# Medical-Image-Analysis-Laboratory/fetal_t2mapping

Measured on AMD Instinct MI355X. Metric: Mvoxel/s T2 fit, 256³×8TE 3-param LM, 1/2/4/8 GPU; % HBM roofline, higher is better.
Workload: dtype f64

## Files before the change

### fetal_t2mapping_amd/csrc/t2fit_boot.hip

```cpp
#include <hip/hip_runtime.h>

#include <chrono>
#include <cmath>
#include <cstdint>
#include <cstdio>
#include <cstdlib>
#include <mutex>
#include <string>
#include <vector>

#include "t2fit_config.h"
#include "t2fit_context.h"
#include "t2fit_error.h"
#include "t2fit_support.h"

namespace {

using t2fit::kBlock;
constexpr int kMaxIntervalReplicas = 512;

__device__ inline void philox4x32_10(uint32_t c0, uint32_t c1, uint32_t c2, uint32_t c3, uint32_t k0, uint32_t k1,
                                     uint32_t& w0, uint32_t& w1) {
#pragma unroll
  for (int round = 0; round < 10; ++round) {
// ... 243 lines not shown
  long long c = 0;
  for (int64_t v = (int64_t)blockIdx.x * kBlock + threadIdx.x; v < n_vox; v += (int64_t)kBgBlocks * kBlock) {
    if (mask[v] != 0) continue;
    for (int j = 0; j < n_te; ++j) {
      const double x = (double)(layout == T2FIT_LAYOUT_TE_MAJOR ? echoes[(int64_t)j * n_vox + v] : echoes[v * n_te + j]);
      s += x * x;
    }
    c += n_te;
  }
  bg_block_reduce(s, c, sh_s, sh_c, part_sum, part_cnt, blockIdx.x);
}

__global__ __launch_bounds__(kBlock) void boot_background_final_kernel(const double* part_sum, const long long* part_cnt,
                                                                       double* out_sum, long long* out_cnt) {
  __shared__ double sh_s[kBlock];
  __shared__ long long sh_c[kBlock];
  double s = 0.0;
  long long c = 0;
  for (int i = threadIdx.x; i < kBgBlocks; i += kBlock) {
    s += part_sum[i];
    c += part_cnt[i];
  }
  bg_block_reduce(s, c, sh_s, sh_c, out_sum, out_cnt, 0);
}

using t2fit::aligned16;
using t2fit::fail;

#ifdef T2FIT_BOOT_PHASES
struct Phases {
  std::chrono::steady_clock::time_point t = std::chrono::steady_clock::now();
  void mark(const char* name) {
    const auto now = std::chrono::steady_clock::now();
    fprintf(stderr, "[t2fit boot phase] %-28s %9.3f ms\n", name, std::chrono::duration<double, std::milli>(now - t).count());
    t = now;
  }
};
#else
struct Phases {
  void mark(const char*) {}
};
#endif

struct BootWorkspace {
  std::vector<void*> dev;
  hipStream_t streams[2] = {nullptr, nullptr};
  bool own_streams = false;
  std::vector<hipEvent_t> events;
  ~BootWorkspace() {
    Phases ph;
    for (hipStream_t s : streams)
      if (s) (void)hipStreamSynchronize(s);
    for (hipEvent_t e : events) (void)hipEventDestroy(e);
    if (own_streams)
      for (hipStream_t s : streams)
        if (s) (void)hipStreamDestroy(s);
    ph.mark("release: sync, events, streams");
    for (void* p : dev) (void)hipFree(p);
    ph.mark("release: hipFree");
  }
  hipError_t alloc(void** p, size_t bytes) {
    const hipError_t e = hipMalloc(p, bytes ? bytes : 16);
    if (e == hipSuccess) dev.push_back(*p);
    return e;
  }
  hipError_t event(hipEvent_t* e) {
    const hipError_t rc = hipEventCreateWithFlags(e, hipEventDisableTiming);
    if (rc == hipSuccess) events.push_back(*e);
    return rc;
  }
};

std::string gib(double bytes) {
  char b[48];
  snprintf(b, sizeof b, "%.2f GiB", bytes / (1024.0 * 1024.0 * 1024.0));
  return b;
}

int synth_check(const char* who, const t2fit_config* cfg, const float* t2_dev, const float* k_dev, double noise_scalar,
                const float* noise_map_dev, int64_t n_vox, int noise_kind) {
  const char* why;
  const int rc = t2fit::config_check(cfg, &why);
  if (rc != T2FIT_OK) return fail(rc, std::string(who) + ": " + why);
  if (cfg->norm)
    return fail(T2FIT_E_INVALID, std::string(who) + ": cfg.norm = 1 is not supported (the maps of a normalised fit are in "
                                 "per-voxel units of the largest sample, and the noise level would have to be too)");
  if (!t2_dev || !k_dev) return fail(T2FIT_E_INVALID, std::string(who) + ": t2_dev / k_dev is NULL");
  if (n_vox < 1 || n_vox >= (1LL << 32)) return fail(T2FIT_E_INVALID, std::string(who) + ": n_vox must be in 1..2^32-1");
  if (noise_kind != T2FIT_BOOT_NOISE_RICIAN && noise_kind != T2FIT_BOOT_NOISE_GAUSSIAN)
    return fail(T2FIT_E_INVALID, std::string(who) + ": unknown noise_kind");
  if (!noise_map_dev && !(noise_scalar >= 0.0 && noise_scalar <= 3.0e38))
    return fail(T2FIT_E_INVALID, std::string(who) + ": noise_scalar must be finite and >= 0 (or give noise_map_dev)");
  return T2FIT_OK;
}

int synth_launch(const t2fit_config* cfg, const float* t2_dev, const float* k_dev, double noise_scalar,
                 const float* noise_map_dev, const uint8_t* mask_dev, int64_t n_vox, int64_t voxel_offset, uint64_t seed,
                 int replica, int noise_kind, float* out, hipStream_t st) {
  SynthArgs a{};
  a.t2 = t2_dev; a.k = k_dev; a.noise_map = noise_map_dev; a.mask = mask_dev; a.out = out;
  a.n_vox = n_vox;
  a.voxel_offset = (uint64_t)voxel_offset;
  a.key0 = (uint32_t)seed; a.key1 = (uint32_t)(seed >> 32); a.replica = (uint32_t)replica;
  a.n_te = cfg->n_te;
  a.noise_scalar = (float)noise_scalar;
  for (int j = 0; j < cfg->n_te; ++j) a.te[j] = (float)cfg->te_ms[j];
  const bool vec = n_vox % 4 == 0 && aligned16(t2_dev) && aligned16(k_dev) && aligned16(out) &&
                   (!noise_map_dev || aligned16(noise_map_dev)) && (reinterpret_cast<uintptr_t>(mask_dev) & 3u) == 0;
  const bool rician = noise_kind == T2FIT_BOOT_NOISE_RICIAN;
// ... 256 lines not shown
```

### fetal_t2mapping_amd/csrc/t2fit_dispatch.h

```cpp
#pragma once

#include "t2fit_lane.h"
#include "t2fit_lbfgsb.h"
#include "t2fit_lm.h"
#include "t2fit_loglin.h"

namespace t2fit {

inline LaneParams make_lane_params(const t2fit_config& c) {
  LaneParams P;
  P.model = c.model; P.solver = c.solver; P.precision = c.precision; P.n_te = c.n_te;
  P.no_prior = c.no_prior; P.norm = c.norm; P.maxls = c.maxls; P.maxiter = c.maxiter;
  P.maxfun = c.maxfun; P.numpy_legacy = c.numpy_legacy != 0;
  for (int i = 0; i < T2FIT_MAX_TE; ++i) {
    P.te[i] = i < c.n_te ? c.te_ms[i] : 0.0;
    P.te_f[i] = (float)P.te[i];
  }
  for (int j = 0; j < 3; ++j) { P.x0[j] = c.x0[j]; P.lb[j] = c.lb[j]; P.ub[j] = c.ub[j]; }
  P.ftol = c.ftol; P.gtol = c.gtol; P.fd_step = c.fd_step; P.lm_xtol = c.lm_xtol;
  P.np_k_ub = c.noprior_k_ub; P.np_t2_lb = c.noprior_t2_lb; P.np_t2_ub = c.noprior_t2_ub;
  P.lm_r_lo = 1.0 / (c.no_prior ? c.noprior_t2_ub : c.ub[1]);
  P.lm_r_hi = 1.0 / (c.no_prior ? c.noprior_t2_lb : c.lb[1]);
  P.lm_r_x0 = 1.0 / c.x0[1];
  t2_exp_res_coefficients(P.exp_c);
  P.inv_n = 1.0 / c.n_te;
  P.te_max = 0.0;
  for (int i = 0; i < c.n_te; ++i) P.te_max = c.te_ms[i] > P.te_max ? c.te_ms[i] : P.te_max;
  P.lbfgsb_tol = (c.ftol / 2.220446049250313e-16) * 2.220446049250313e-16;
  return P;
}

struct LaneOutputs {
  float t2, k, sigma, res, r2, fun, se;
  int32_t nit;
  uint8_t status;
};

T2_HD ObjCtx prepare_samples(const LaneParams& P, float* col, int stride, bool& finite, float& y0_raw) {
  const int n = P.n_te;
  finite = true;
  y0_raw = col[0];
  float ymax = col[0];
  for (int i = 0; i < n; ++i) {
    const float v = col[i * stride];
    finite = finite && t2_finite(v);
    ymax = v > ymax ? v : ymax;
  }
  if (P.norm) {
    for (int i = 0; i < n; ++i) {
      const float v = col[i * stride] / ymax;
      col[i * stride] = v;
      finite = finite && t2_finite(v);
    }
  }
  ObjCtx c;
  c.P = &P;
  c.y = EchoView{col, stride};
  return c;
}

template <int SOLVER, int PREC, int MODEL>
T2_HD void fit_lane_t(const LaneParams& P, const ObjCtx& c, bool finite, float y0_raw, LaneResult& r) {
  constexpr int NP = MODEL == T2FIT_MODEL_GAUSSIAN ? 2 : 3;
  double lb[3], ub[3];
  const bool feasible = lane_bounds(P, y0_raw, lb, ub);
  r.nit = 0;
  r.nfev = 0;
  r.fun = NAN;
  if (!feasible) {
    r.x[0] = r.x[1] = NAN;
    r.x[2] = NP == 2 ? 0.0 : NAN;
    r.status = T2FIT_ST_INFEASIBLE;
    return;
  }
  if (!finite) {
    for (int j = 0; j < 3; ++j) r.x[j] = j < NP ? t2_clip(P.x0[j], lb[j], ub[j]) : 0.0;
    r.status = T2FIT_ST_NONFINITE;
    return;
  }
  if constexpr (SOLVER == T2FIT_SOLVER_LOGLIN) {
    static_assert(MODEL == T2FIT_MODEL_GAUSSIAN, "the log-linear closed form exists for the 2-parameter model only");
    loglin_solve(c, lb, ub, true, r);
  } else if constexpr (SOLVER == T2FIT_SOLVER_LM) {
    static_assert(MODEL != T2FIT_MODEL_RICIAN, "LM handles the least-squares models only");
    if constexpr (PREC == T2FIT_PREC_F32) lm_solve<float, NP>(c, lb, ub, r);
    else lm_solve<double, NP>(c, lb, ub, r);
  } else {
    lbfgsb_solve<MODEL>(c, lb, ub, r);
  }
}

T2_HD float r_squared(const ObjCtx& c, double k, double t2, double sg) {
  const LaneParams& P = *c.P;
  const int n = P.n_te;
  double mean = 0.0;
  for (int i = 0; i < n; ++i) mean += (double)c.sample(i);
  mean /= n;
  double ss_tot = 0.0, ss_res = 0.0;
  const bool sq = P.model == T2FIT_MODEL_GAUSSIAN_RICIAN;
  for (int i = 0; i < n; ++i) {
    const double yi = (double)c.sample(i);
    const double E = t2_exp(-P.te[i] / t2);
    const double m = sq ? t2_sqrt(k * k * E * E + sg * sg) : k * E;
    ss_res += (yi - m) * (yi - m);
    ss_tot += (yi - mean) * (yi - mean);
  }
  return (float)(1.0 - ss_res / ss_tot);
}

T2_HD float t2_std_error(const ObjCtx& c, double k, double t2, double sg) {
  const LaneParams& P = *c.P;
  const int n = P.n_te;
  const bool sq = P.model == T2FIT_MODEL_GAUSSIAN_RICIAN;
  const int np = P.model == T2FIT_MODEL_GAUSSIAN ? 2 : 3;
  if (n <= np) return NAN;
  double a00 = 0, a01 = 0, a02 = 0, a11 = 0, a12 = 0, a22 = 0, ss = 0;
  for (int i = 0; i < n; ++i) {
    const double t = P.te[i];
    const double E = t2_exp(-t / t2);
    double m, jk, jt, js;
    if (sq) {
      m = t2_sqrt(k * k * E * E + sg * sg);
      jk = k * E * E / m;
      jt = k * k * E * E * (t / (t2 * t2)) / m;
      js = sg / m;
    } else {
      m = k * E;
      jk = E;
      jt = m * t / (t2 * t2);
      js = 0.0;
    }
    const double r = (double)c.sample(i) - m;
    ss += r * r;
    a00 += jk * jk; a01 += jk * jt; a02 += jk * js; a11 += jt * jt; a12 += jt * js; a22 += js * js;
  }
  const double s2 = ss / (n - np);
  double var;
  if (sq) {
    const double det = a00 * (a11 * a22 - a12 * a12) - a01 * (a01 * a22 - a12 * a02) + a02 * (a01 * a12 - a11 * a02);
    var = s2 * (a00 * a22 - a02 * a02) / det;
  } else if (np == 3) {
    var = s2 * a00 / (a00 * a11 - a01 * a01);
  } else {
    var = s2 * a00 / (a00 * a11 - a01 * a01);
  }
  return var > 0.0 ? (float)t2_sqrt(var) : NAN;
}

T2_HD void lane_epilogue(const ObjCtx& c, const LaneResult& r, LaneOutputs& o, bool want_r2, bool want_se) {
  o.k = (float)r.x[0];
  o.t2 = (float)r.x[1];
  o.sigma = (float)r.x[2];
  o.fun = (float)r.fun;
  o.nit = r.nit;
  o.status = r.status;
  o.res = residual_mean(c, o.k, o.t2, o.sigma);
  o.r2 = want_r2 ? r_squared(c, (double)o.k, (double)o.t2, (double)o.sigma) : 0.0f;
  o.se = want_se ? t2_std_error(c, (double)o.k, (double)o.t2, (double)o.sigma) : 0.0f;
}

}
```

### fetal_t2mapping_amd/csrc/t2fit_kernels.hip

```cpp
#include <hip/hip_runtime.h>

#include <algorithm>
#include <atomic>
#include <cstdlib>
#include <string>

#include "t2fit_config.h"
#include "t2fit_diag.h"
#include "t2fit_dispatch.h"
#include "t2fit_error.h"
#include "t2fit_launch.h"
#include "t2fit_support.h"

using namespace t2fit;

namespace {

constexpr int kLdsStride = kBlock + 1;
#ifndef T2_SAMPLE_LOAD
#define T2_SAMPLE_LOAD(p) (*(p))
#endif
#ifndef T2_WAVE_HINT
#define T2_WAVE_HINT 2
#endif
constexpr int kWaveHint = T2_WAVE_HINT;

struct Tuning {
  bool use_persistent = true;
  int persistent_blocks = 2048;
  int refill_min = 0;
  bool nte_special = true;
  int take = 0;
  int64_t small_volume = 1 << 20;
  int wave_wg = 1;
  int waves_per_cu = 0;
};
std::atomic<bool> g_reserve_set{false};
std::atomic<int> g_reserve_cus{0};

const Tuning& tuning() {
  static const Tuning tuned = [] {
    Tuning t;
    if (const char* e = std::getenv("T2FIT_ONE_SHOT")) t.use_persistent = std::atoi(e) == 0;
    if (const char* e = std::getenv("T2FIT_PERSISTENT_BLOCKS")) t.persistent_blocks = std::max(1, std::atoi(e));
    if (const char* e = std::getenv("T2FIT_REFILL_MIN")) t.refill_min = std::min(64, std::max(1, std::atoi(e)));
    if (const char* e = std::getenv("T2FIT_RESERVE_CUS"); e && !g_reserve_set.load()) g_reserve_cus.store(std::max(0, std::atoi(e)));
    if (const char* e = std::getenv("T2FIT_NTE_SPECIAL")) t.nte_special = std::atoi(e) != 0;
    if (const char* e = std::getenv("T2FIT_TAKE")) t.take = std::max(0, std::min(64, std::atoi(e)));
    if (const char* e = std::getenv("T2FIT_SMALL_VOLUME")) t.small_volume = std::max<int64_t>(0, std::atoll(e));
    if (const char* e = std::getenv("T2FIT_WAVE_WG")) t.wave_wg = std::max(0, std::atoi(e));
    if (const char* e = std::getenv("T2FIT_WAVES_PER_CU")) t.waves_per_cu = std::max(0, std::atoi(e));
    return t;
  }();
  return tuned;
}

thread_local bool g_timing = false;
constexpr int kEvRing = 16;
thread_local hipEvent_t g_ev0[kEvRing] = {}, g_ev1[kEvRing] = {}, g_ev2[kEvRing] = {};
thread_local long g_ev_count = 0;
thread_local int g_ev_slot = 0;

double event_ms(int launches_ago, const hipEvent_t* from, const hipEvent_t* to) {
  if (launches_ago < 0 || launches_ago >= kEvRing || launches_ago >= g_ev_count) return -1.0;
  const int slot = (int)((g_ev_count - 1 - launches_ago) % kEvRing);
  if (hipEventSynchronize(to[slot]) != hipSuccess) return -1.0;
  float ms = 0.0f;
  if (hipEventElapsedTime(&ms, from[slot], to[slot]) != hipSuccess) return -1.0;
  return (double)ms;
}

struct DevMaps {
  float *t2, *k, *sigma, *res, *r2, *fun, *se;
  int32_t* nit;
  uint8_t* status;
  double* xd;
  double* fund;
  double* trace = nullptr;
  int32_t* trace_len = nullptr;
  int trace_cap = 0;
};

__device__ __forceinline__ void stage_echoes(float* lds, const float* __restrict__ echoes, int layout,
                                             int n_te, int64_t n_vox, int64_t base, bool load_own) {
  const int lane = threadIdx.x;
  if (layout == T2FIT_LAYOUT_TE_MAJOR) {
    if (load_own) {
      const float* src = echoes + base + lane;
      for (int i = 0; i < n_te; ++i) lds[i * kLdsStride + lane] = src[(int64_t)i * n_vox];
    }
  } else {
    const int64_t rows = n_vox - base < kBlock ? n_vox - base : kBlock;
    const int total = (int)rows * n_te;
    const float* src = echoes + base * n_te;
    for (int j = lane; j < total; j += kBlock) {
      const int v = j / n_te;
      const int i = j - v * n_te;
      lds[i * kLdsStride + v] = src[j];
    }
    __syncthreads();
  }
}

template <bool kExtras = true, bool kEpilogueFollows = false>
__device__ __forceinline__ void store_masked(const DevMaps& m, int64_t v) {
  m.t2[v] = 0.0f; m.k[v] = 0.0f; m.sigma[v] = 0.0f;
  if constexpr (!kEpilogueFollows) m.res[v] = 0.0f;
  if constexpr (!kExtras) return;
// ... 457 lines not shown
        busy = false;
        done = true;
      }
    }
  }
  if (done) {
    LaneResult r;
    A::result(s, c, r);
    store_fit<kExtras>(m, v, r);
  }
  T2_STAMPS_END(next_chunk, lane)
}

template <class A, int kChunk, bool kTrace = false, int kWavesPerSimd = 1, bool kExtras = true, int kWg = kBlock,
          bool kRegs = false>
__global__ __launch_bounds__(kWg, kWavesPerSimd) void fit_persistent_kernel(const LaneParams P,
                                                                    const float* __restrict__ echoes, int layout,
                                                                    const uint8_t* __restrict__ mask, int64_t n_vox,
                                                                    DevMaps m, unsigned long long* next_chunk, int refill_min,
                                                                    int take, double* ghist) {
  persistent_fit<A, kChunk, kTrace, kExtras, kWg, kRegs>(P, echoes, layout, mask, n_vox, m, next_chunk, refill_min, take, ghist,
                                                         (KernargParams)__builtin_amdgcn_kernarg_segment_ptr());
}

__global__ __launch_bounds__(kBlock) void residuals_kernel(const LaneParams P, const float* __restrict__ echoes,
                                                           int layout, const uint8_t* __restrict__ mask,
                                                           int64_t n_vox, const float* __restrict__ t2,
                                                           const float* __restrict__ k,
                                                           const float* __restrict__ sigma, float* res, float* r2,
                                                           float* se) {
  extern __shared__ float lds[];
  const int lane = threadIdx.x;
  const int64_t base = (int64_t)blockIdx.x * kBlock;
  const int64_t v = base + lane;
  const bool in_range = v < n_vox;
  const bool active = in_range && (mask == nullptr || mask[v] != 0);
  stage_echoes(lds, echoes, layout, P.n_te, n_vox, base, active);
  if (!in_range) return;
  float out = 0.0f, out2 = 0.0f, out3 = 0.0f;
  if (active) {
    bool finite;
    float y0_raw;
    const ObjCtx c = prepare_samples(P, lds + lane, kLdsStride, finite, y0_raw);
    const float kv = k[v], tv = t2[v], sv = sigma ? sigma[v] : 0.0f;
    out = residual_mean(c, kv, tv, sv);
    if (r2) out2 = r_squared(c, (double)kv, (double)tv, (double)sv);
    if (se) out3 = t2_std_error(c, (double)kv, (double)tv, (double)sv);
  }
  res[v] = out;
  if (r2) r2[v] = out2;
  if (se) se[v] = out3;
}

using FitKernel = void (*)(const LaneParams, const float*, int, const uint8_t*, int64_t, DevMaps);

FitKernel pick_kernel(const t2fit_config& c) {
  if (c.solver == T2FIT_SOLVER_LM) {
    if (c.precision == T2FIT_PREC_F32)
      return c.model == T2FIT_MODEL_GAUSSIAN
                 ? fit_volume_kernel<T2FIT_SOLVER_LM, T2FIT_PREC_F32, T2FIT_MODEL_GAUSSIAN>
                 : fit_volume_kernel<T2FIT_SOLVER_LM, T2FIT_PREC_F32, T2FIT_MODEL_GAUSSIAN_RICIAN>;
    return c.model == T2FIT_MODEL_GAUSSIAN
               ? fit_volume_kernel<T2FIT_SOLVER_LM, T2FIT_PREC_F64, T2FIT_MODEL_GAUSSIAN>
               : fit_volume_kernel<T2FIT_SOLVER_LM, T2FIT_PREC_F64, T2FIT_MODEL_GAUSSIAN_RICIAN>;
  }
  if (c.solver == T2FIT_SOLVER_LOGLIN)
    return fit_volume_kernel<T2FIT_SOLVER_LOGLIN, T2FIT_PREC_F64, T2FIT_MODEL_GAUSSIAN>;
  return nullptr;
}

bool wants_extras(const DevMaps& dm) { return dm.r2 || dm.se || dm.fun || dm.nit || dm.status || dm.xd || dm.fund; }

struct LaunchArgs {
  unsigned grid; size_t lds_samples; hipStream_t st;
  const LaneParams& P; const float* echoes; int layout; const uint8_t* mask; int64_t n_vox; const DevMaps& dm;
  unsigned long long* counter;
  bool big;
};

template <class A, bool kLargeOnly = false, bool kWaveOnly = false>
hipError_t launch_persistent(const LaunchArgs& a) {
  constexpr int W = A::kWavesPerSimd;
  const Tuning& tune = tuning();
  const DevMaps& dm = a.dm;
  const bool extras = wants_extras(dm);
  const int refill_min = tune.refill_min > 0 ? tune.refill_min : A::kRefillMin;
  if constexpr (!kPhaseStamps && kLargeOnly && A::kHistDoubles > 0 && A::kWaveWgOk) {
    if (tune.wave_wg) {
      using AW = typename A::WaveWg;
      constexpr int kHint = AW::kWaveWgHint;
      auto k64 = extras ? fit_persistent_kernel<AW, kChunkSmall, false, kHint, true, 64, true>
                        : fit_persistent_kernel<AW, kChunkSmall, false, kHint, false, 64, true>;
      unsigned wg = 64;
      if constexpr (kWgShapeDiag) {
        if (tune.wave_wg == 2) { k64 = fit_persistent_kernel<AW, kChunkSmall, false, 1, false, 256, true>; wg = 256; }
        if (tune.wave_wg == 3) { k64 = fit_persistent_kernel<AW, kChunkSmall, false, 1, false, 128, true>; wg = 128; }
      }
      size_t lds64 = (size_t)AW::kHistDoubles * wg * sizeof(double);
      unsigned per_cu = (unsigned)std::min<size_t>(wg == 64 ? 4 * kHint : 512 / wg, 128 / ceil_div<size_t>(lds64, 1280));
      if (tune.waves_per_cu > 0 && (unsigned)tune.waves_per_cu < per_cu) {
        per_cu = (unsigned)tune.waves_per_cu;
        lds64 = (size_t)(128 / per_cu) * 1280;
      }
      hipError_t e = hipFuncSetAttribute(reinterpret_cast<const void*>(k64), hipFuncAttributeMaxDynamicSharedMemorySize,
                                         (int)lds64);
      if (e != hipSuccess) return e;
// ... 15 lines not shown
    return hipErrorNotSupported;
  } else {
    auto kern = extras ? fit_persistent_kernel<A, kChunkLarge, false, W, true>
                       : fit_persistent_kernel<A, kChunkLarge, false, W, false>;
    if constexpr (!kLargeOnly) {
      if (dm.trace) kern = fit_persistent_kernel<A, kChunkSmall, true, W>;
      else if (!a.big) kern = fit_persistent_kernel<A, kChunkSmall, false, W>;
    }
    const size_t lds = ((a.lds_samples / sizeof(float) + 1) & ~(size_t)1) * sizeof(float) +
                       (size_t)A::kHistDoubles * kBlock * sizeof(double) +
                       (size_t)(kBlock / 64) * (kQueueCap * sizeof(uint32_t) + kStampLdsBytesPerWave);
    hipError_t e = hipFuncSetAttribute(reinterpret_cast<const void*>(kern), hipFuncAttributeMaxDynamicSharedMemorySize,
                                       (int)lds);
    if (e != hipSuccess) return e;
    hipLaunchKernelGGL(kern, dim3(a.grid), dim3(kBlock), lds, a.st, a.P, a.echoes, a.layout, a.mask, a.n_vox, dm, a.counter,
                       refill_min, 1, (double*)nullptr);
    return hipGetLastError();
  }
}

template <int MODEL>
hipError_t launch_lbfgsb(int n_te, const LaunchArgs& a) {
  if (a.big && tuning().nte_special) {
    if (n_te == 8) return launch_persistent<LbfgsbLane<MODEL, 8>, true>(a);
    if (n_te == 6) return launch_persistent<LbfgsbLane<MODEL, 6>, true>(a);
    if (n_te == 3) return launch_persistent<LbfgsbLane<MODEL, 3>, true>(a);
    hipError_t e = hipErrorNotSupported;
    if (tuning().wave_wg == 1) {
      if (n_te == 7) e = launch_persistent<LbfgsbLane<MODEL, 7>, true, true>(a);
      if (n_te == 5) e = launch_persistent<LbfgsbLane<MODEL, 5>, true, true>(a);
      if (n_te == 4) e = launch_persistent<LbfgsbLane<MODEL, 4>, true, true>(a);
    }
    if (e != hipErrorNotSupported) return e;
  }
  return launch_persistent<LbfgsbLane<MODEL>>(a);
}

template <int NPAR>
hipError_t launch_lm_f64(int n_te, const LaunchArgs& a) {
  if (a.big && tuning().nte_special) {
    if (n_te == 8) return launch_persistent<LmLaneAdaptor<double, NPAR, 8>, true>(a);
    if (n_te == 6) return launch_persistent<LmLaneAdaptor<double, NPAR, 6>, true>(a);
    if (n_te == 3) return launch_persistent<LmLaneAdaptor<double, NPAR, 3>, true>(a);
  }
  return launch_persistent<LmLaneAdaptor<double, NPAR>>(a);
}

bool loglin_vec_ok(const float* echoes, int layout, const uint8_t* mask, int64_t n_vox, const DevMaps& dm, int n_te) {
  return layout == T2FIT_LAYOUT_TE_MAJOR && n_vox % kLoglinVec == 0 && aligned16(echoes) &&
         (reinterpret_cast<uintptr_t>(mask) & 3u) == 0 && aligned16(dm.t2) && aligned16(dm.k) && aligned16(dm.sigma) &&
         aligned16(dm.res) && (size_t)n_te * kLoglinTile * sizeof(float) <= 65536;
}

}

int t2fit::check_common(const t2fit_config* cfg, const void* echoes, int layout, int64_t n_vox) {
  const char* why;
  const int rc = config_check(cfg, &why);
  if (rc != T2FIT_OK) return fail(rc, why);
  if (!echoes) return fail(T2FIT_E_INVALID, "echoes is NULL");
  if (layout != T2FIT_LAYOUT_TE_MAJOR && layout != T2FIT_LAYOUT_VOXEL_MAJOR) return fail(T2FIT_E_INVALID, "unknown layout");
  if (n_vox < 0) return fail(T2FIT_E_INVALID, "n_vox is negative");
  if (ceil_div<int64_t>(n_vox, kBlock) > 0x7fffffffLL) return fail(T2FIT_E_INVALID, "n_vox too large for one launch");
  return T2FIT_OK;
}

bool t2fit::is_large_volume(int64_t n_vox) { return n_vox > tuning().small_volume; }

int t2fit::launch_fit(const t2fit_config* cfg, const float* echoes, int layout, const uint8_t* mask, int64_t n_vox,
                      const t2fit_maps& maps, hipStream_t st, bool part_of_large, const VoxelOutputs& vox) {
  if (n_vox == 0) return T2FIT_OK;
  const DevMaps dm{maps.t2, maps.k, maps.sigma, maps.res, maps.r2, maps.fun, maps.t2_se, maps.nit, maps.status,
                   vox.xd, vox.fund, vox.trace, vox.trace_len, vox.trace_cap};
  const Tuning& tune = tuning();
  const LaneParams P = make_lane_params(*cfg);
  const unsigned grid = (unsigned)ceil_div<int64_t>(n_vox, kBlock);
  const size_t lds = (size_t)cfg->n_te * kLdsStride * sizeof(float);
  FitKernel kern = pick_kernel(*cfg);
  const bool loglin = cfg->solver == T2FIT_SOLVER_LOGLIN;
  const bool persistent = !loglin && (tune.use_persistent || cfg->solver == T2FIT_SOLVER_LBFGSB);
  if (persistent && n_vox >= 0xffffffffLL) return fail(T2FIT_E_INVALID, "n_vox must be below 2^32 per call");
  unsigned long long* counter = nullptr;
  if (persistent) {
    T2_HIP(hipMallocAsync((void**)&counter, kCounterWords * sizeof(unsigned long long), st));
    T2_HIP(hipMemsetAsync(counter, 0, kCounterWords * sizeof(unsigned long long), st));
  }
  if (g_timing) {
    g_ev_slot = (int)(g_ev_count % kEvRing);
    if (!g_ev0[g_ev_slot]) {
      T2_HIP(hipEventCreate(&g_ev0[g_ev_slot]));
      T2_HIP(hipEventCreate(&g_ev1[g_ev_slot]));
      T2_HIP(hipEventCreate(&g_ev2[g_ev_slot]));
    }
    T2_HIP(hipEventRecord(g_ev0[g_ev_slot], st));
  }
  if (persistent) {
    const bool big = !dm.trace && (part_of_large || is_large_volume(n_vox));
    const int64_t chunks = ceil_div<int64_t>(n_vox, big ? kChunkLarge : kChunkSmall);
    unsigned pgrid = (unsigned)std::min<int64_t>((chunks + 3) / 4, tune.persistent_blocks);
    const int reserve = g_reserve_cus.load(std::memory_order_relaxed);
    if (reserve > 0 && cfg->solver == T2FIT_SOLVER_LBFGSB) {
      int dev = 0, cus = 0;
      T2_HIP(hipGetDevice(&dev));
      T2_HIP(hipDeviceGetAttribute(&cus, hipDeviceAttributeMultiprocessorCount, dev));
      pgrid = std::min<unsigned>(pgrid, (unsigned)std::max(1, cus - reserve));
    }
    const LaunchArgs a{pgrid, lds, st, P, echoes, layout, mask, n_vox, dm, counter, big};
    const bool two = cfg->model == T2FIT_MODEL_GAUSSIAN;
    hipError_t pe;
    if (cfg->solver == T2FIT_SOLVER_LBFGSB) {
      if (two) pe = launch_lbfgsb<T2FIT_MODEL_GAUSSIAN>(cfg->n_te, a);
      else if (cfg->model == T2FIT_MODEL_GAUSSIAN_RICIAN) pe = launch_lbfgsb<T2FIT_MODEL_GAUSSIAN_RICIAN>(cfg->n_te, a);
      else pe = launch_lbfgsb<T2FIT_MODEL_RICIAN>(cfg->n_te, a);
    } else if (cfg->precision == T2FIT_PREC_F32) {
      pe = two ? launch_persistent<LmLaneAdaptor<float, 2>>(a) : launch_persistent<LmLaneAdaptor<float, 3>>(a);
    } else {
      pe = two ? launch_lm_f64<2>(cfg->n_te, a) : launch_lm_f64<3>(cfg->n_te, a);
    }
    if (pe != hipSuccess) {
      (void)hipFreeAsync(counter, st);
      return fail(T2FIT_E_HIP, std::string("persistent fit launch: ") + hipGetErrorString(pe));
    }
    if (g_timing) T2_HIP(hipEventRecord(g_ev1[g_ev_slot], st));
    hipLaunchKernelGGL(residuals_kernel, dim3(grid), dim3(kBlock), lds, st, P, echoes, layout, mask, n_vox,
                       (const float*)dm.t2, (const float*)dm.k, (const float*)dm.sigma, dm.res, dm.r2, dm.se);
    if (g_timing) {
      T2_HIP(hipEventRecord(g_ev2[g_ev_slot], st));
      ++g_ev_count;
    }
  } else if (loglin && loglin_vec_ok(echoes, layout, mask, n_vox, dm, cfg->n_te)) {
    hipLaunchKernelGGL(wants_extras(dm) ? loglin_volume_kernel<true> : loglin_volume_kernel<false>,
                       dim3((unsigned)ceil_div<int64_t>(n_vox, kLoglinTile)), dim3(kBlock),
                       (size_t)cfg->n_te * kLoglinTile * sizeof(float), st, P, echoes, mask, n_vox, dm);
  } else {
    hipLaunchKernelGGL(kern, dim3(grid), dim3(kBlock), lds, st, P, echoes, layout, mask, n_vox, dm);
  }
  T2_HIP(hipGetLastError());
  if (g_timing && !persistent) {
    T2_HIP(hipEventRecord(g_ev1[g_ev_slot], st));
    T2_HIP(hipEventRecord(g_ev2[g_ev_slot], st));
    ++g_ev_count;
  }
  if (counter && cfg->solver == T2FIT_SOLVER_LBFGSB) {
    if (const int rc = report_stamps(counter, st)) return rc;
    if (const int rc = report_placement(counter, st)) return rc;
  }
  if (counter) T2_HIP(hipFreeAsync(counter, st));
  return T2FIT_OK;
}

extern "C" {

int t2fit_set_reserve_cus(int cus) {
  g_reserve_set.store(true);
  return g_reserve_cus.exchange(std::max(0, cus));
}

int t2fit_set_timing(int enabled) {
  g_timing = enabled != 0;
  g_ev_count = 0;
  return T2FIT_OK;
}

double t2fit_kernel_ms(int launches_ago) { return event_ms(launches_ago, g_ev0, g_ev1); }

double t2fit_last_kernel_ms(void) { return t2fit_kernel_ms(0); }

double t2fit_epilogue_ms(int launches_ago) { return event_ms(launches_ago, g_ev1, g_ev2); }

int t2fit_volume_dev(const t2fit_config* cfg, const float* echoes_dev, int layout, const uint8_t* mask_dev,
                     int64_t n_vox, const t2fit_maps* maps, void* stream) {
  int rc = check_common(cfg, echoes_dev, layout, n_vox);
  if (rc != T2FIT_OK) return rc;
  if (!maps || !maps->t2 || !maps->k || !maps->sigma || !maps->res)
    return fail(T2FIT_E_INVALID, "maps->t2/k/sigma/res must be non-NULL");
  return launch_fit(cfg, echoes_dev, layout, mask_dev, n_vox, *maps, (hipStream_t)stream);
}

int t2fit_residuals_dev(const t2fit_config* cfg, const float* echoes_dev, int layout, const uint8_t* mask_dev,
                        int64_t n_vox, const float* t2, const float* k, const float* sigma, float* res, void* stream) {
  int rc = check_common(cfg, echoes_dev, layout, n_vox);
  if (rc != T2FIT_OK) return rc;
  if (!t2 || !k || !res) return fail(T2FIT_E_INVALID, "t2/k/res must be non-NULL");
  if (n_vox == 0) return T2FIT_OK;
  const LaneParams P = make_lane_params(*cfg);
  const unsigned grid = (unsigned)ceil_div<int64_t>(n_vox, kBlock);
  const size_t lds = (size_t)cfg->n_te * kLdsStride * sizeof(float);
  hipLaunchKernelGGL(residuals_kernel, dim3(grid), dim3(kBlock), lds, (hipStream_t)stream, P, echoes_dev, layout,
                     mask_dev, n_vox, t2, k, sigma, res, (float*)nullptr, (float*)nullptr);
  T2_HIP(hipGetLastError());
  return T2FIT_OK;
}

}
```

### fetal_t2mapping_amd/csrc/t2fit_lane.h

```cpp
#pragma once

#include <math.h>
#include <stdint.h>

#include <type_traits>

#include "../../include/t2fit.h"
#include "t2fit_diag.h"

#if defined(__HIPCC__)
#define T2_HD __host__ __device__ __forceinline__
#define T2_DEVICE_COMPILE 1
#define T2_UNROLL _Pragma("unroll")
#else
#define T2_HD inline
#define T2_UNROLL
#endif

namespace t2fit {

struct LaneParams {
  int32_t model, solver, precision, n_te;
  int32_t no_prior, norm, maxls, maxiter, maxfun, numpy_legacy;
  double te[T2FIT_MAX_TE];
// ... 392 lines not shown
}
#if defined(T2_OCML_LOG)
#define T2_LOG_I0E(v) t2_log(v)
#else
#define T2_LOG_I0E(v) t2_log_lean(v)
#endif

T2_HD void t2_log_i0e4(const double* x, double* out, bool near = false) {
  double ax[4], z[4], ra[4], rb[4], r[4];
  bool small[4];
  T2_UNROLL
  for (int j = 0; j < 4; ++j) {
    ax[j] = x[j] < 0 ? -x[j] : x[j];
    small[j] = ax[j] <= 8.0;
    ra[j] = 0.0;
    rb[j] = 0.0;
  }
  const bool any_small = small[0] || small[1] || small[2] || small[3];
  const bool any_large = !(small[0] && small[1] && small[2] && small[3]);
#if defined(T2_I0E_STATS) && !defined(__HIPCC__)
  ++g_calls; g_small += any_small; g_large += any_large;
#endif
  const bool wave_small = T2_WAVE_ANY(any_small), wave_large = T2_WAVE_ANY(any_large);
  if (wave_small && wave_large && !T2_WAVE_ANY(any_small && any_large)) {
    t2_i0e4_by_lane(ax, any_small, r, near);
  } else {
    if (wave_small) {
      T2_UNROLL
      for (int j = 0; j < 4; ++j) z[j] = ax[j] * 0.5 - 2.0;
      t2_chbevl4(z, t2_i0e_A, 6, ra);
    }
    if (wave_large) {
      T2_UNROLL
      for (int j = 0; j < 4; ++j) z[j] = t2_fdiv(32.0, ax[j]) - 2.0;
      t2_chbevl4(z, t2_i0e_B, 5, rb);
      T2_UNROLL
      for (int j = 0; j < 4; ++j) rb[j] = t2_fdiv(rb[j], t2_sqrt_core(ax[j]));
    }
    T2_UNROLL
    for (int j = 0; j < 4; ++j) r[j] = small[j] ? ra[j] : rb[j];
  }
  T2_UNROLL
  for (int j = 0; j < 4; ++j) out[j] = T2_LOG_I0E(r[j]);
}

struct ObjCtx {
  const LaneParams* P;
  EchoView y;
  double* trace = nullptr;
  int trace_cap = 0;
  int* trace_n = nullptr;
  T2_DIAG_COUNTERS
  T2_HD float sample(int i) const { return y[i]; }
};


T2_HD int n_params(int model) { return model == T2FIT_MODEL_GAUSSIAN ? 2 : 3; }

T2_HD bool lane_bounds(const LaneParams& P, float y0_raw, double* lb, double* ub) {
  for (int j = 0; j < 3; ++j) {
    lb[j] = P.lb[j];
    ub[j] = P.ub[j];
  }
  if (P.no_prior) {
    lb[0] = (double)y0_raw;
    ub[0] = P.np_k_ub;
    lb[1] = P.np_t2_lb;
    ub[1] = P.np_t2_ub;
  }
  const int np = n_params(P.model);
  bool ok = true;
  for (int j = 0; j < np; ++j) ok = ok && !(lb[j] > ub[j]);
  return ok;
}

T2_HD double t2_exp_res(double x, const double* cc) {
  const double n = nearbyint(x * 1.4426950408889634);
  double r = fma(n, -6.93147180369123816490e-01, x);
  r = fma(n, -1.90821492927058770002e-10, r);
  double p = cc[0];
#if defined(T2_DEVICE_COMPILE)
#pragma unroll
#endif
  for (int j = 1; j < 10; ++j) p = fma(p, r, cc[j]);
  p = fma(p, r, 1.0);
  p = fma(p, r, 1.0);
  const double nc = fmin(fmax(n, -2000.0), 2000.0);
  return x < -746.0 ? 0.0 : ldexp(p, (int)nc);
}
inline void t2_exp_res_coefficients(double* cc) {
  double f = 1.0;
  for (int j = 2; j <= 11; ++j) { f *= j; cc[11 - j] = 1.0 / f; }
}

T2_HD float residual_mean(const ObjCtx& c, float k32, float t232, float s32) {
  const int n = c.P->n_te;
  const bool gauss = c.P->model == T2FIT_MODEL_GAUSSIAN;
  const bool legacy = c.P->numpy_legacy != 0;
  const double k = (double)k32, t2 = (double)t232;
  const double k2 = (double)(k32 * k32), s2 = (double)(s32 * s32);
  const double rt2 = 1.0 / t2;
  auto resid = [&](int i) {
    const double te = c.P->te[i];
    if (legacy) {
      const float pf = gauss ? k32 * expf((float)(-te) / t232)
                             : sqrtf((k32 * k32) * expf((float)(-2.0 * te) / t232) + s32 * s32);
      return c.sample(i) - pf;
    }
    double pred;
    if (gauss) pred = k * t2_exp_res(t2_div_by_rcp(-te, t2, rt2), c.P->exp_c);
    else pred = t2_sqrt(k2 * t2_exp_res(t2_div_by_rcp(-2.0 * te, t2, rt2), c.P->exp_c) + s2);
    return c.sample(i) - (float)pred;
  };
  if (n == 8) {
    float r[8];
#if defined(T2_DEVICE_COMPILE)
#pragma unroll
#endif
    for (int i = 0; i < 8; ++i) r[i] = resid(i);
    return (((r[0] + r[1]) + (r[2] + r[3])) + ((r[4] + r[5]) + (r[6] + r[7]))) / 8.0f;
  }
  if (n < 8) {
    float sum = 0.0f;
    for (int i = 0; i < n; ++i) sum += resid(i);
    return sum / (float)n;
  }
  float r8[8] = {0, 0, 0, 0, 0, 0, 0, 0};
  float sum = 0.0f;
  const int n8 = n & ~7;
  for (int i = 0; i < n; ++i) {
    const float r = resid(i);
    if (i >= n8) {
      if (i == n8) sum = ((r8[0] + r8[1]) + (r8[2] + r8[3])) + ((r8[4] + r8[5]) + (r8[6] + r8[7]));
      sum += r;
    } else {
      const int slot = i & 7;
#if defined(T2_DEVICE_COMPILE)
#pragma unroll
#endif
      for (int j = 0; j < 8; ++j) r8[j] = (j == slot) ? r8[j] + r : r8[j];
    }
  }
  if (n8 == n) sum = ((r8[0] + r8[1]) + (r8[2] + r8[3])) + ((r8[4] + r8[5]) + (r8[6] + r8[7]));
  return sum / (float)n;
}

}
```

### fetal_t2mapping_amd/csrc/t2fit_lbfgsb.h

```cpp
#pragma once

#include <type_traits>

#include "t2fit_lane.h"

namespace t2fit {

template <int MODEL> struct ObjTerm;
T2_HD double rician_log_term(float log_y, double log_s2, bool legacy) {
  return legacy ? (double)(log_y - (float)log_s2) : (double)log_y - log_s2;
}
template <> struct ObjTerm<T2FIT_MODEL_GAUSSIAN> {
  double k, t2;
  T2_HD void set(const ObjCtx&, const double* x) { k = x[0]; t2 = x[1]; }
  T2_HD double at(const ObjCtx& c, int i) const {
    const double r = (double)c.sample(i) - k * t2_exp_core(t2_fdiv(-c.P->te[i], t2));
    return r * r;
  }
  T2_HD double finish(const ObjCtx& c, double s) const { return s / c.P->n_te; }
};
template <> struct ObjTerm<T2FIT_MODEL_GAUSSIAN_RICIAN> {
  double k2, t2, s2;
  T2_HD void set(const ObjCtx&, const double* x) { k2 = x[0] * x[0]; t2 = x[1]; s2 = x[2] * x[2]; }
  T2_HD double at(const ObjCtx& c, int i) const {
// ... 747 lines not shown
      for (int i = 0; i < N; ++i) {
        if (fr[i]) {
          const double dk = du[i];
          if (dk < 0.0) {
            const double temp2 = lb[i] - z[i];
            if (temp2 >= 0.0) temp1 = 0.0;
            else if (dk * alpha < temp2) temp1 = t2_fdiv(temp2, dk);
          } else if (dk > 0.0) {
            const double temp2 = ub[i] - z[i];
            if (temp2 <= 0.0) temp1 = 0.0;
            else if (dk * alpha > temp2) temp1 = t2_fdiv(temp2, dk);
          }
          if (temp1 < alpha) {
            alpha = temp1;
            T2_UNROLL
            for (int j = 0; j < N; ++j) hit[j] = j == i;
          }
        }
      }
      if (alpha < 1.0) {
        T2_UNROLL
        for (int i = 0; i < N; ++i)
          if (hit[i]) {
            if (du[i] > 0.0) { z[i] = ub[i]; du[i] = 0.0; }
            else if (du[i] < 0.0) { z[i] = lb[i]; du[i] = 0.0; }
          }
      }
      T2_UNROLL
      for (int i = 0; i < N; ++i)
        if (fr[i]) z[i] = fma(alpha, du[i], z[i]);
    }
    return pos_def;
  }

  T2_HD void init(const double* x0_, const double* lb_, const double* ub_, double* hist_, int hstride_,
                  double* ghist_ = nullptr, int gstride_ = 0) {
    hist = hist_;
    hstride = hstride_;
    ghist = ghist_;
    gstride = gstride_;
    head = 0;
    T2_UNROLL
    for (int i = 0; i < N; ++i) {
      lb[i] = lb_[i];
      ub[i] = ub_[i];
      x[i] = t2_clip(x0_[i], lb[i], ub[i]);
      iwhere[i] = (ub[i] - lb[i] <= 0.0) ? 3 : 0;
    }
    col = 0; nit = 0; nfev = 0; ifun = 0;
    theta = 1.0;
    status = T2FIT_ST_NOT_CONV;
    first = true;
    wn_stale = false;
    T2_UNROLL
    for (int i = 0; i < N; ++i) { z[i] = 0.0; d[i] = 0.0; t[i] = 0.0; r[i] = 0.0; g[i] = 0.0; }
    f = 0.0; fold = 0.0; gd = 0.0; gdold = 0.0; stp = 1.0; stpmx = 1.0; sbgnrm = 0.0;
    ls.task = LS_START; ls.stage = 1; ls.brackt = false;
    ls.ginit = ls.gtest = ls.gx = ls.gy = ls.finit = ls.fx = ls.fy = 0.0;
    ls.stx = ls.sty = ls.stmin = ls.stmax = ls.width = ls.width1 = 0.0;
  }

  enum { GO_BEGIN, GO_TRIAL, GO_FAIL, GO_DONE };

  T2_HD int digest(const ObjCtx& c) {
    const LaneParams& P = *c.P;
    const double epsmch = 2.220446049250313e-16;
    T2_BLK_T0(t_dig)
    const bool was_first = first;
    first = false;
    double gdn = 0.0;
    T2_UNROLL
    for (int i = 0; i < N; ++i) gdn += g[i] * d[i];
    LsState lsn = ls;
    const int task = dcsrch_tests(f, gdn, stp, 0.9, 0.1, 0.0, stpmx, lsn);
    const bool cont = !was_first & (task == LS_FG);
    const bool newit = !was_first & (task != LS_FG);
    double stpn = stp;
    dcsrch_update(f, gdn, stpn, 0.1, 0.0, stpmx, lsn);
    const double sb = projgr(x, g);
    const double tol = P.lbfgsb_tol;
    const int nit1 = nit + 1;
    const bool out_of_budget = (nit1 >= P.maxiter) | (nfev > P.maxfun);
    const bool converged = (sb <= P.gtol) | (!was_first & ((fold - f) <= tol * t2_max3(lb_abs(fold), lb_abs(f), 1.0)));
    double rn[N], dn[N], rr = 0.0;
    T2_UNROLL
    for (int i = 0; i < N; ++i) { rn[i] = g[i] - r[i]; rr += rn[i] * rn[i]; }
    const double dr = (gdn - gdold) * stp, ddum = -gdold * stp;
    T2_UNROLL
    for (int i = 0; i < N; ++i) dn[i] = d[i] * stp;
    const double theta_n = t2_fdiv(rr, dr);
    const double rsy = t2_fast_rsqrt(dr);
    const bool iterate_on = newit & !out_of_budget & !converged;
    const bool store_pair = iterate_on & !(dr <= epsmch * ddum);
    if (!was_first) gd = gdn;
    if (cont) { ls = lsn; stp = stpn; ++ifun; }
    if (!cont && !was_first) ls.task = lsn.task;
    if (was_first || newit) sbgnrm = sb;
    if (newit) {
      nit = nit1;
      if (c.trace && *c.trace_n < c.trace_cap) {
        double* tr = c.trace + 4 * (*c.trace_n)++;
        tr[0] = x[0]; tr[1] = x[1]; tr[2] = N == 3 ? x[N - 1] : 0.0; tr[3] = f;
      }
    }
    if (iterate_on) {
      T2_UNROLL
      for (int i = 0; i < N; ++i) { r[i] = rn[i]; d[i] = dn[i]; }
    }
    if (store_pair) {
      if (col == M) {
        head = (head + 1) % M;
        col = M - 1;
// ... 126 lines not shown
```

### fetal_t2mapping_amd/csrc/t2fit_support.h

```cpp
#pragma once

#include <hip/hip_runtime.h>

#include <cstddef>
#include <cstdint>
#include <mutex>
#include <string>
#include <vector>

#include "t2fit_error.h"

namespace t2fit {

constexpr int kBlock = 256;

inline bool aligned16(const void* p) { return (reinterpret_cast<uintptr_t>(p) & 15u) == 0; }
inline bool misaligned(const void* p, uintptr_t a) { return (reinterpret_cast<uintptr_t>(p) & (a - 1)) != 0; }
constexpr size_t align_up(size_t v, size_t a) { return (v + a - 1) / a * a; }
template <class T> constexpr T ceil_div(T a, T b) { return (a + b - 1) / b; }

inline int check_workspace(const std::string& who, const void* ws, size_t bytes, size_t need, const char* bytes_fn) {
  if (!ws) return fail(T2FIT_E_INVALID, who + ": workspace_dev is NULL");
  if (misaligned(ws, 256)) return fail(T2FIT_E_INVALID, who + ": workspace_dev is not aligned to 256 bytes");
  if (bytes < need)
    return fail(T2FIT_E_INVALID, who + ": workspace too small: " + std::to_string(bytes) + " bytes given, " + std::to_string(need) + " needed (" +
                                     bytes_fn + ")");
  return T2FIT_OK;
}

__device__ inline double wave_butterfly(double v) {
#pragma unroll
  for (int s = 32; s >= 1; s >>= 1) v = v + __shfl_xor(v, s, 64);
  return v;
}

__device__ inline bool finite_bits(float v) { return (__float_as_uint(v) & 0x7f800000u) != 0x7f800000u; }

enum ScratchUse : int {
  kScratchRing,
  kScratchRoiErode,
  kScratchRoiStats,
  kScratchComponents,
};
struct ScratchCache {
  struct Entry { int device; hipStream_t stream; int use; void* p; size_t bytes; };
  std::mutex mutex;
  std::vector<Entry> entries;
  static ScratchCache& get() { static ScratchCache c; return c; }
};

template <class T> hipError_t scratch_get(hipStream_t st, ScratchUse use, size_t bytes, T** out) {
  int dev = 0;
  hipError_t e = hipGetDevice(&dev);
  if (e != hipSuccess) return e;
  ScratchCache& cache = ScratchCache::get();
  std::lock_guard<std::mutex> g(cache.mutex);
  ScratchCache::Entry* r = nullptr;
  for (ScratchCache::Entry& c : cache.entries)
    if (c.device == dev && c.stream == st && c.use == use) r = &c;
  if (!r) {
    cache.entries.push_back(ScratchCache::Entry{dev, st, use, nullptr, 0});
    r = &cache.entries.back();
  }
  if (r->bytes < bytes) {
    if (r->p) {
      if ((e = hipStreamSynchronize(st)) != hipSuccess) return e;
      (void)hipFree(r->p);
      r->p = nullptr;
      r->bytes = 0;
    }
    if ((e = hipMalloc(&r->p, bytes)) != hipSuccess) return e;
    r->bytes = bytes;
  }
  *out = static_cast<T*>(r->p);
  return hipSuccess;
}

inline void scratch_release_stream(int device, hipStream_t st) {
  ScratchCache& cache = ScratchCache::get();
  std::lock_guard<std::mutex> g(cache.mutex);
  for (size_t i = cache.entries.size(); i-- > 0;)
    if (cache.entries[i].device == device && cache.entries[i].stream == st) {
      if (cache.entries[i].p) (void)hipFree(cache.entries[i].p);
      cache.entries.erase(cache.entries.begin() + i);
    }
}

}
```

Before: 1664.

## Add vectorized TE-major residual kernel and cache the persistent counter buffer

Adds a residuals kernel for TE-major layout in which each thread handles four voxels. It uses float4 loads, keeps samples in registers with a compile-time echo count, and writes results with float4 stores, avoiding the LDS staging path. The persistent-fit counter now comes from a per-stream scratch cache guarded by a mutex instead of a hipMallocAsync/hipFreeAsync pair on every call, and owned streams release their scratch entries on teardown. It also drops the zero-initialisation of L-BFGS-B state arrays in reset, which risks reads of uninitialised values if any path depends on them.

```diff
diff --git a/fetal_t2mapping_amd/csrc/t2fit_boot.hip b/fetal_t2mapping_amd/csrc/t2fit_boot.hip
--- a/fetal_t2mapping_amd/csrc/t2fit_boot.hip
+++ b/fetal_t2mapping_amd/csrc/t2fit_boot.hip
@@ -319,9 +319,15 @@
     for (hipStream_t s : streams)
       if (s) (void)hipStreamSynchronize(s);
     for (hipEvent_t e : events) (void)hipEventDestroy(e);
-    if (own_streams)
+    if (own_streams) {
+      int device = 0;
+      const bool have_device = hipGetDevice(&device) == hipSuccess;
       for (hipStream_t s : streams)
-        if (s) (void)hipStreamDestroy(s);
+        if (s) {
+          if (have_device) t2fit::scratch_release_stream(device, s);
+          (void)hipStreamDestroy(s);
+        }
+    }
     ph.mark("release: sync, events, streams");
     for (void* p : dev) (void)hipFree(p);
     ph.mark("release: hipFree");
diff --git a/fetal_t2mapping_amd/csrc/t2fit_dispatch.h b/fetal_t2mapping_amd/csrc/t2fit_dispatch.h
--- a/fetal_t2mapping_amd/csrc/t2fit_dispatch.h
+++ b/fetal_t2mapping_amd/csrc/t2fit_dispatch.h
@@ -59,6 +59,28 @@
   return c;
 }
 
+template <int NTE>
+T2_HD void prepare_samples(const LaneParams& P, RegSamples<NTE>& c, bool& finite, float& y0_raw) {
+  finite = true;
+  y0_raw = c.y[0];
+  float ymax = c.y[0];
+  T2_UNROLL
+  for (int i = 0; i < NTE; ++i) {
+    const float v = c.y[i];
+    finite = finite && t2_finite(v);
+    ymax = v > ymax ? v : ymax;
+  }
+  if (P.norm) {
+    T2_UNROLL
+    for (int i = 0; i < NTE; ++i) {
+      const float v = c.y[i] / ymax;
+      c.y[i] = v;
+      finite = finite && t2_finite(v);
+    }
+  }
+  c.P = &P;
+}
+
 template <int SOLVER, int PREC, int MODEL>
 T2_HD void fit_lane_t(const LaneParams& P, const ObjCtx& c, bool finite, float y0_raw, LaneResult& r) {
   constexpr int NP = MODEL == T2FIT_MODEL_GAUSSIAN ? 2 : 3;
@@ -90,9 +112,10 @@
   }
 }
 
-T2_HD float r_squared(const ObjCtx& c, double k, double t2, double sg) {
+template <class Ctx>
+T2_HD float r_squared(const Ctx& c, double k, double t2, double sg) {
   const LaneParams& P = *c.P;
-  const int n = P.n_te;
+  const int n = c.n_te();
   double mean = 0.0;
   for (int i = 0; i < n; ++i) mean += (double)c.sample(i);
   mean /= n;
@@ -108,9 +131,10 @@
   return (float)(1.0 - ss_res / ss_tot);
 }
 
-T2_HD float t2_std_error(const ObjCtx& c, double k, double t2, double sg) {
+template <class Ctx>
+T2_HD float t2_std_error(const Ctx& c, double k, double t2, double sg) {
   const LaneParams& P = *c.P;
-  const int n = P.n_te;
+  const int n = c.n_te();
   const bool sq = P.model == T2FIT_MODEL_GAUSSIAN_RICIAN;
   const int np = P.model == T2FIT_MODEL_GAUSSIAN ? 2 : 3;
   if (n <= np) return NAN;
diff --git a/fetal_t2mapping_amd/csrc/t2fit_kernels.hip b/fetal_t2mapping_amd/csrc/t2fit_kernels.hip
--- a/fetal_t2mapping_amd/csrc/t2fit_kernels.hip
+++ b/fetal_t2mapping_amd/csrc/t2fit_kernels.hip
@@ -54,6 +54,8 @@
   }();
   return tuned;
 }
+
+std::mutex g_counter_mutex;
 
 thread_local bool g_timing = false;
 constexpr int kEvRing = 16;
@@ -617,6 +619,57 @@
   if (se) se[v] = out3;
 }
 
+constexpr int kResVec = 4;
+constexpr int kResTile = kBlock * kResVec;
+
+template <int NTE, bool kExtras>
+__global__ __launch_bounds__(kBlock) void residuals_te_major_kernel(const LaneParams P, const float* __restrict__ echoes,
+                                                                    const uint8_t* __restrict__ mask, int64_t n_vox,
+                                                                    const float* __restrict__ t2,
+                                                                    const float* __restrict__ k,
+                                                                    const float* __restrict__ sigma, float* res,
+                                                                    float* r2, float* se) {
+  const int64_t v0 = (int64_t)blockIdx.x * kResTile + (int64_t)threadIdx.x * kResVec;
+  if (v0 >= n_vox) return;
+  bool act[kResVec] = {true, true, true, true};
+  if (mask) {
+    const uchar4 mk = *reinterpret_cast<const uchar4*>(mask + v0);
+    act[0] = mk.x != 0; act[1] = mk.y != 0; act[2] = mk.z != 0; act[3] = mk.w != 0;
+  }
+  float out[kResVec] = {0.0f, 0.0f, 0.0f, 0.0f}, out2[kResVec] = {0.0f, 0.0f, 0.0f, 0.0f},
+        out3[kResVec] = {0.0f, 0.0f, 0.0f, 0.0f};
+  if (act[0] || act[1] || act[2] || act[3]) {
+    float4 s[NTE];
+#pragma unroll
+    for (int i = 0; i < NTE; ++i) s[i] = *reinterpret_cast<const float4*>(echoes + (int64_t)i * n_vox + v0);
+    const float4 k4 = *reinterpret_cast<const float4*>(k + v0);
+    const float4 t4 = *reinterpret_cast<const float4*>(t2 + v0);
+    const float4 s4 = sigma ? *reinterpret_cast<const float4*>(sigma + v0) : make_float4(0.0f, 0.0f, 0.0f, 0.0f);
+    const float kq[kResVec] = {k4.x, k4.y, k4.z, k4.w}, tq[kResVec] = {t4.x, t4.y, t4.z, t4.w},
+                sq[kResVec] = {s4.x, s4.y, s4.z, s4.w};
+#pragma unroll
+    for (int q = 0; q < kResVec; ++q) {
+      if (!act[q]) continue;
+      RegSamples<NTE> c;
+#pragma unroll
+      for (int i = 0; i < NTE; ++i) c.y[i] = q == 0 ? s[i].x : q == 1 ? s[i].y : q == 2 ? s[i].z : s[i].w;
+      bool finite;
+      float y0_raw;
+      prepare_samples(P, c, finite, y0_raw);
+      out[q] = residual_mean(c, kq[q], tq[q], sq[q]);
+      if constexpr (kExtras) {
+        if (r2) out2[q] = r_squared(c, (double)kq[q], (double)tq[q], (double)sq[q]);
+        if (se) out3[q] = t2_std_error(c, (double)kq[q], (double)tq[q], (double)sq[q]);
+      }
+    }
+  }
+  *reinterpret_cast<float4*>(res + v0) = make_float4(out[0], out[1], out[2], out[3]);
+  if constexpr (kExtras) {
+    if (r2) *reinterpret_cast<float4*>(r2 + v0) = make_float4(out2[0], out2[1], out2[2], out2[3]);
+    if (se) *reinterpret_cast<float4*>(se + v0) = make_float4(out3[0], out3[1], out3[2], out3[3]);
+  }
+}
+
 using FitKernel = void (*)(const LaneParams, const float*, int, const uint8_t*, int64_t, DevMaps);
 
 FitKernel pick_kernel(const t2fit_config& c) {
@@ -738,6 +791,41 @@
          aligned16(dm.res) && (size_t)n_te * kLoglinTile * sizeof(float) <= 65536;
 }
 
+struct ResidualArgs {
+  const float* echoes; int layout; const uint8_t* mask; int64_t n_vox;
+  const float *t2, *k, *sigma;
+  float *res, *r2, *se;
+};
+
+bool residuals_vec_ok(const ResidualArgs& a, int n_te) {
+  return a.layout == T2FIT_LAYOUT_TE_MAJOR && n_te >= 3 && n_te <= 8 && a.n_vox % kResVec == 0 && aligned16(a.echoes) &&
+         (reinterpret_cast<uintptr_t>(a.mask) & 3u) == 0 && aligned16(a.t2) && aligned16(a.k) && aligned16(a.sigma) &&
+         aligned16(a.res) && aligned16(a.r2) && aligned16(a.se);
+}
+
+template <int NTE>
+void launch_residuals_te_major(const LaneParams& P, const ResidualArgs& a, hipStream_t st) {
+  auto kern = a.r2 || a.se ? residuals_te_major_kernel<NTE, true> : residuals_te_major_kernel<NTE, false>;
+  hipLaunchKernelGGL(kern, dim3((unsigned)ceil_div<int64_t>(a.n_vox, kResTile)), dim3(kBlock), 0, st, P, a.echoes, a.mask,
+                     a.n_vox, a.t2, a.k, a.sigma, a.res, a.r2, a.se);
+}
+
+void launch_residuals(const LaneParams& P, const ResidualArgs& a, hipStream_t st) {
+  if (residuals_vec_ok(a, P.n_te)) {
+    switch (P.n_te) {
+      case 3: return launch_residuals_te_major<3>(P, a, st);
+      case 4: return launch_residuals_te_major<4>(P, a, st);
+      case 5: return launch_residuals_te_major<5>(P, a, st);
+      case 6: return launch_residuals_te_major<6>(P, a, st);
+      case 7: return launch_residuals_te_major<7>(P, a, st);
+      default: return launch_residuals_te_major<8>(P, a, st);
+    }
+  }
+  hipLaunchKernelGGL(residuals_kernel, dim3((unsigned)ceil_div<int64_t>(a.n_vox, kBlock)), dim3(kBlock),
+                     (size_t)P.n_te * kLdsStride * sizeof(float), st, P, a.echoes, a.layout, a.mask, a.n_vox, a.t2, a.k,
+                     a.sigma, a.res, a.r2, a.se);
+}
+
 }
 
 int t2fit::check_common(const t2fit_config* cfg, const void* echoes, int layout, int64_t n_vox) {
@@ -767,8 +855,10 @@
   const bool persistent = !loglin && (tune.use_persistent || cfg->solver == T2FIT_SOLVER_LBFGSB);
   if (persistent && n_vox >= 0xffffffffLL) return fail(T2FIT_E_INVALID, "n_vox must be below 2^32 per call");
   unsigned long long* counter = nullptr;
+  std::unique_lock<std::mutex> counter_lock;
   if (persistent) {
-    T2_HIP(hipMallocAsync((void**)&counter, kCounterWords * sizeof(unsigned long long), st));
+    T2_HIP(scratch_get(st, kScratchCounter, kCounterWords * sizeof(unsigned long long), &counter));
+    counter_lock = std::unique_lock<std::mutex>(g_counter_mutex);
     T2_HIP(hipMemsetAsync(counter, 0, kCounterWords * sizeof(unsigned long long), st));
   }
   if (g_timing) {
@@ -803,13 +893,10 @@
     } else {
       pe = two ? launch_lm_f64<2>(cfg->n_te, a) : launch_lm_f64<3>(cfg->n_te, a);
     }
-    if (pe != hipSuccess) {
-      (void)hipFreeAsync(counter, st);
-      return fail(T2FIT_E_HIP, std::string("persistent fit launch: ") + hipGetErrorString(pe));
-    }
+    if (pe != hipSuccess) return fail(T2FIT_E_HIP, std::string("persistent fit launch: ") + hipGetErrorString(pe));
+    if constexpr (!kPhaseStamps && !kWgShapeDiag) counter_lock.unlock();
     if (g_timing) T2_HIP(hipEventRecord(g_ev1[g_ev_slot], st));
-    hipLaunchKernelGGL(residuals_kernel, dim3(grid), dim3(kBlock), lds, st, P, echoes, layout, mask, n_vox,
-                       (const float*)dm.t2, (const float*)dm.k, (const float*)dm.sigma, dm.res, dm.r2, dm.se);
+    launch_residuals(P, ResidualArgs{echoes, layout, mask, n_vox, dm.t2, dm.k, dm.sigma, dm.res, dm.r2, dm.se}, st);
     if (g_timing) {
       T2_HIP(hipEventRecord(g_ev2[g_ev_slot], st));
       ++g_ev_count;
@@ -831,7 +918,6 @@
     if (const int rc = report_stamps(counter, st)) return rc;
     if (const int rc = report_placement(counter, st)) return rc;
   }
-  if (counter) T2_HIP(hipFreeAsync(counter, st));
   return T2FIT_OK;
 }
 
@@ -870,10 +956,8 @@
   if (!t2 || !k || !res) return fail(T2FIT_E_INVALID, "t2/k/res must be non-NULL");
   if (n_vox == 0) return T2FIT_OK;
   const LaneParams P = make_lane_params(*cfg);
-  const unsigned grid = (unsigned)ceil_div<int64_t>(n_vox, kBlock);
-  const size_t lds = (size_t)cfg->n_te * kLdsStride * sizeof(float);
-  hipLaunchKernelGGL(residuals_kernel, dim3(grid), dim3(kBlock), lds, (hipStream_t)stream, P, echoes_dev, layout,
-                     mask_dev, n_vox, t2, k, sigma, res, (float*)nullptr, (float*)nullptr);
+  launch_residuals(P, ResidualArgs{echoes_dev, layout, mask_dev, n_vox, t2, k, sigma, res, nullptr, nullptr},
+                   (hipStream_t)stream);
   T2_HIP(hipGetLastError());
   return T2FIT_OK;
 }
diff --git a/fetal_t2mapping_amd/csrc/t2fit_lane.h b/fetal_t2mapping_amd/csrc/t2fit_lane.h
--- a/fetal_t2mapping_amd/csrc/t2fit_lane.h
+++ b/fetal_t2mapping_amd/csrc/t2fit_lane.h
@@ -468,6 +468,14 @@
   int* trace_n = nullptr;
   T2_DIAG_COUNTERS
   T2_HD float sample(int i) const { return y[i]; }
+  T2_HD int n_te() const { return P->n_te; }
+};
+
+template <int NTE> struct RegSamples {
+  const LaneParams* P;
+  float y[NTE];
+  T2_HD float sample(int i) const { return y[i]; }
+  T2_HD constexpr int n_te() const { return NTE; }
 };
 
 
@@ -509,8 +517,9 @@
   for (int j = 2; j <= 11; ++j) { f *= j; cc[11 - j] = 1.0 / f; }
 }
 
-T2_HD float residual_mean(const ObjCtx& c, float k32, float t232, float s32) {
-  const int n = c.P->n_te;
+template <class Ctx>
+T2_HD float residual_mean(const Ctx& c, float k32, float t232, float s32) {
+  const int n = c.n_te();
   const bool gauss = c.P->model == T2FIT_MODEL_GAUSSIAN;
   const bool legacy = c.P->numpy_legacy != 0;
   const double k = (double)k32, t2 = (double)t232;
diff --git a/fetal_t2mapping_amd/csrc/t2fit_lbfgsb.h b/fetal_t2mapping_amd/csrc/t2fit_lbfgsb.h
--- a/fetal_t2mapping_amd/csrc/t2fit_lbfgsb.h
+++ b/fetal_t2mapping_amd/csrc/t2fit_lbfgsb.h
@@ -823,12 +823,7 @@
     status = T2FIT_ST_NOT_CONV;
     first = true;
     wn_stale = false;
-    T2_UNROLL
-    for (int i = 0; i < N; ++i) { z[i] = 0.0; d[i] = 0.0; t[i] = 0.0; r[i] = 0.0; g[i] = 0.0; }
-    f = 0.0; fold = 0.0; gd = 0.0; gdold = 0.0; stp = 1.0; stpmx = 1.0; sbgnrm = 0.0;
     ls.task = LS_START; ls.stage = 1; ls.brackt = false;
-    ls.ginit = ls.gtest = ls.gx = ls.gy = ls.finit = ls.fx = ls.fy = 0.0;
-    ls.stx = ls.sty = ls.stmin = ls.stmax = ls.width = ls.width1 = 0.0;
   }
 
   enum { GO_BEGIN, GO_TRIAL, GO_FAIL, GO_DONE };
diff --git a/fetal_t2mapping_amd/csrc/t2fit_support.h b/fetal_t2mapping_amd/csrc/t2fit_support.h
--- a/fetal_t2mapping_amd/csrc/t2fit_support.h
+++ b/fetal_t2mapping_amd/csrc/t2fit_support.h
@@ -38,6 +38,7 @@
 
 enum ScratchUse : int {
   kScratchRing,
+  kScratchCounter,
   kScratchRoiErode,
   kScratchRoiStats,
   kScratchComponents,
```

New measurement: 1680 (median of 6 runs). No clear change (+1.0%).
